# robertvoy/ComfyUI-Distributed

Hardware: AMD Instinct MI355X
Metric: tiles/sec (whole node), sd15 USDU 4x->4096 512px tiles (higher is better)
Workload: dtype bf16; 1 GPU; model=sd15-unet-860M-random-init, global_batch=1, canvas=4096x4096, tile=512+pad32->544, tiles_per_image=64, sampler=euler/20steps/denoise0.5/cfg8.0, parallelism=tile-pull-queue dp1 over RCCL/xGMI

## Files before the change

comfyui_distributed_amd/ops/hip/bindings.cpp:

```cpp
#include <torch/extension.h>

torch::Tensor group_norm_fused(torch::Tensor x, int64_t groups,
                               torch::Tensor weight, torch::Tensor bias,
                               double eps, bool fuse_silu);
torch::Tensor layer_norm_bf16(torch::Tensor x, torch::Tensor gamma,
                              torch::Tensor beta, double eps);
torch::Tensor act_mul_bf16(torch::Tensor a, torch::Tensor b, bool gelu);
torch::Tensor extract_resize(torch::Tensor src, int64_t x1, int64_t y1,
                             int64_t x2, int64_t y2, int64_t ow, int64_t oh);
void blend_tile(torch::Tensor canvas, torch::Tensor tile, int64_t x1,
                int64_t y1, int64_t x2, int64_t y2, int64_t mx1, int64_t my1,
                int64_t mx2, int64_t my2, double sigma);
torch::Tensor attn_fwd(torch::Tensor q, torch::Tensor k, torch::Tensor v,
                       int64_t heads, int64_t kv_heads, int64_t nk_real,
                       double scale);
torch::Tensor attn_fwd_packed(torch::Tensor q, torch::Tensor k,
                              torch::Tensor v, int64_t heads,
                              int64_t kv_heads, double scale);
torch::Tensor attn_fwd_qkv(torch::Tensor qkv, int64_t heads, double scale);
torch::Tensor attn_fwd_q_kv(torch::Tensor q, torch::Tensor kv, int64_t heads,
                            double scale);
torch::Tensor mfma_selftest(torch::Tensor a, torch::Tensor b);
torch::Tensor conv_nhwc(torch::Tensor x, torch::Tensor wt, torch::Tensor bias,
                        int64_t B, int64_t H, int64_t W, int64_t C, int64_t K,
                        int64_t rs, bool fuse_silu);
torch::Tensor group_norm_nhwc(torch::Tensor x, int64_t groups,
                              torch::Tensor weight, torch::Tensor bias,
                              double eps, bool fuse_silu,
                              c10::optional<torch::Tensor> addend);
std::vector<int64_t> group_norm_nhwc_plan(int64_t B, int64_t HW, int64_t C);
torch::Tensor conv_smallc(torch::Tensor x, torch::Tensor wt, torch::Tensor bias,
                          int64_t B, int64_t H, int64_t W, int64_t C,
                          int64_t K, int64_t rs, bool fuse_silu);
torch::Tensor gemm256_bf16(torch::Tensor x, torch::Tensor w,
                           torch::Tensor bias, bool fuse_silu);
torch::Tensor conv256_nhwc(torch::Tensor x, torch::Tensor wt,
                           torch::Tensor bias, torch::Tensor residual,
                           int64_t B, int64_t H,
                           int64_t W, int64_t C, int64_t K, int64_t rs,
                           int64_t stride, bool up2, bool fuse_silu);
torch::Tensor conv256_nhwc_ex(torch::Tensor x, torch::Tensor wt,
                              torch::Tensor bias, torch::Tensor residual,
                              int64_t B, int64_t H,
                              int64_t W, int64_t C, int64_t K, int64_t rs,
                              int64_t stride, bool up2, bool fuse_silu,
                              int64_t bn, int64_t split_k);
std::tuple<int64_t, int64_t> conv256_plan(int64_t M, int64_t K_out,
                                          int64_t Kdim);
void qk_norm_rope(torch::Tensor q, torch::Tensor k, torch::Tensor q_weight,
                  torch::Tensor k_weight, torch::Tensor cos, torch::Tensor sin,
                  torch::Tensor out_q, torch::Tensor out_k, int64_t heads,
                  double eps, int64_t token_offset);
torch::Tensor norm_modulate(torch::Tensor x, torch::Tensor weight,
                            torch::Tensor scale, torch::Tensor shift,
                            double eps);
std::tuple<torch::Tensor, torch::Tensor> norm_modulate_fp8(
    torch::Tensor x, torch::Tensor weight, torch::Tensor scale,
    torch::Tensor shift, double eps);
torch::Tensor gated_residual(torch::Tensor x, torch::Tensor gate,
                             torch::Tensor y);
std::tuple<torch::Tensor, torch::Tensor> quant_rows_fp8(torch::Tensor x);
torch::Tensor gemm_fp8(torch::Tensor qa, torch::Tensor sa, torch::Tensor qw,
                       torch::Tensor sw, torch::Tensor bias, int64_t act);

PYBIND11_MODULE(TORCH_EXTENSION_NAME, m) {
  m.def("group_norm_fused", &group_norm_fused,
        "fused GroupNorm(+SiLU), NCHW bf16");
  m.def("layer_norm", &layer_norm_bf16, "LayerNorm over last dim, bf16");
  m.def("act_mul", &act_mul_bf16, "a * act(b) elementwise, bf16");
  m.def("extract_resize", &extract_resize,
        "crop region of [B,H,W,C] f32 -> Lanczos-3 resample");
  m.def("blend_tile", &blend_tile,
        "fused resample + blurred-rect mask + composite (in-place canvas)");
  m.def("attn_fwd", &attn_fwd, "flash attention forward, bf16 MFMA");
  m.def("attn_fwd_packed", &attn_fwd_packed,
        "flash attention on packed [B,N,H*D] QKV (no host reshapes)");
  m.def("attn_fwd_qkv", &attn_fwd_qkv,
        "self-attention on fused [B,N,3*H*D] projection output");
  m.def("attn_fwd_q_kv", &attn_fwd_q_kv,
        "cross-attention on q [B,Nq,H*D] + fused kv [B,Nk,2*H*D]");
  m.def("mfma_selftest", &mfma_selftest,
        "single-wave 16x16x32 bf16 MFMA with the kernel fragment layouts");
  m.def("conv_nhwc", &conv_nhwc,
        "implicit-GEMM 3x3/1x1 NHWC bf16 conv on MFMA (+fused SiLU)");
  m.def("group_norm_nhwc", &group_norm_nhwc,
        "fused GroupNorm(+SiLU), NHWC bf16; addend [B, C] bf16 is added per "
        "sample (rounded to bf16) before the statistics",
        py::arg("x"), py::arg("groups"), py::arg("weight"), py::arg("bias"),
        py::arg("eps"), py::arg("fuse_silu"), py::arg("addend") = py::none());
  m.def("group_norm_nhwc_plan", &group_norm_nhwc_plan,
        "(B, HW, C) -> (threads, pixels per step, slots per lane, blocks per "
        "image, pixels per block) of the two-pass NHWC GroupNorm; launches "
        "nothing");
  m.def("conv_smallc", &conv_smallc,
        "small-C NHWC conv (stem convs, C <= 8)");
  m.def("gemm256_bf16", &gemm256_bf16,
        "256x256x64 glds-staged MFMA GEMM, torch-Linear layout (+SiLU)");
  m.def("conv256_nhwc", &conv256_nhwc,
        "256-tile implicit-GEMM 3x3/1x1 NHWC conv on the same template; "
        "N-tile width and K split chosen per call");
  m.def("conv256_nhwc_ex", &conv256_nhwc_ex,
        "conv256_nhwc with the variant pinned: bn in {128, 256, 320} and "
        "split_k (clamped to the K-tile count); 0 = chooser");
  m.def("conv256_plan", &conv256_plan,
        "(M, K_out, Kdim) -> (bn, split_k) the conv launcher picks; "
        "launches nothing");
  m.def("qk_norm_rope", &qk_norm_rope,
        "per-head RMSNorm + RoPE of strided q/k views into [B,Ntot,H*D] "
        "buffers at a token offset");
  m.def("norm_modulate", &norm_modulate,
        "row RMSNorm (fp32 weight) or affine-free LayerNorm (empty weight) "
        "+ optional adaLN (1+scale)/shift");
  m.def("norm_modulate_fp8", &norm_modulate_fp8,
        "quant_rows_fp8(norm_modulate(...)) in one launch -> (float8_e4m3fn "
        "[B,N,C], fp32 row scale [B,N]); C % 128 == 0, C <= 8192");
  m.def("gated_residual", &gated_residual, "x + gate[b] * y, bf16");
  m.def("quant_rows_fp8", &quant_rows_fp8,
        "bf16 [M,K] -> (float8_e4m3fn [M,K], fp32 row scale [M] = amax/448)");
  m.def("gemm_fp8", &gemm_fp8,
        "act((qa . qw^T) * sa[m] * sw[n] + bias[n]) -> bf16 on the block-"
        "scaled 16x16x128 MFMA; act 0 none, 1 SiLU, 2 GELU-tanh");
}
```

comfyui_distributed_amd/ops/hip/gemm.hip:

```cpp

#include <torch/extension.h>
#include <ATen/hip/HIPContext.h>
#include "gemm_tile.h"

#define GBM TILE_BM
#define GBN 256
#define GBK 64

struct ConvGeo {
  int H, W, C;
  int Ho, Wo;
  int stride;
  int up2;
  int RS;
  int tile2d;
  int xcd_swz;
};

__device__ __forceinline__ unsigned xcd_remap(unsigned id, unsigned nwg) {
  const unsigned q = nwg / 8u, r = nwg % 8u;
  const unsigned xcd = id % 8u, pos = id / 8u;
  return (xcd < r ? xcd * (q + 1u) : r * (q + 1u) + (xcd - r) * q) + pos;
}

template <bool IS_CONV>
struct AChunk {
  typename std::conditional<IS_CONV, unsigned, long long>::type off;
  int yx;
};
#define A_ROW_DEAD 0x7fff0001

template <bool IS_CONV, bool FUSE_SILU, int BN, bool SPLITK>
__global__ __launch_bounds__(512, 1) void gemm256_kernel(
    const uint16_t* __restrict__ A,
    const uint16_t* __restrict__ Bw,
    const float* __restrict__ bias,
    const uint16_t* __restrict__ zero_page,
    const uint16_t* __restrict__ residual,
    uint16_t* __restrict__ Y,
    float* __restrict__ ws,
    long long M, int N, int Kdim, ConvGeo geo) {
  static_assert(BN == 128 || BN == 256 || BN == 320, "unsupported N-tile");
  constexpr int NF = BN / 64;
  constexpr int NB = BN / 64;
  constexpr unsigned B_TILE = BN * 128u;
  const TileThread t = tile_thread();
  const int wave = t.wave, wm = t.wm, wn = t.wn, fr = t.fr, kgrp = t.kgrp,
            r0 = t.r0;

  __shared__ __align__(16) uint16_t lds[32768 + BN * 128];
  uint8_t* const lds8 = reinterpret_cast<uint8_t*>(lds);

  unsigned bx = blockIdx.x;
  if (IS_CONV && geo.xcd_swz) bx = xcd_remap(bx, gridDim.x);
  long long m_blk = 0;
  int t_b = 0, t_py0 = 0, t_px0 = 0;
  if (IS_CONV && geo.tile2d) {
    const int tx_n = geo.Wo >> 4;
    const int per_img = tx_n * (geo.Ho >> 4);
    t_b = (int)(bx / per_img);
    const int rem = (int)(bx % per_img);
    t_py0 = (rem / tx_n) << 4;
    t_px0 = (rem % tx_n) << 4;
  } else {
    m_blk = (long long)bx * GBM;
  }
  const int n_blk = blockIdx.y * BN;

  const int c_loc = (int)(t.c_byte >> 1);
  const int bn0 = n_blk + r0;
  const long long b_off = (long long)bn0 * Kdim + c_loc;
  AChunk<IS_CONV> a_desc[2][2];
#pragma unroll
  for (int i = 0; i < 2; ++i) {
#pragma unroll
    for (int pc = 0; pc < 2; ++pc) {
      const int m_local = t.a_row(0, pc, i);
      AChunk<IS_CONV> d;
      if (IS_CONV) {
        long long img;
        int py, px;
        bool ok = true;
        if (geo.tile2d) {
          py = t_py0 + (m_local >> 4);
          px = t_px0 + (m_local & 15);
          img = (long long)t_b * geo.H * geo.W * geo.C;
        } else {
          const long long m = m_blk + m_local;
          ok = m < M;
          const long long HWo = (long long)geo.Ho * geo.Wo;
          const long long mm = ok ? m : 0;
          const int pb = (int)(mm / HWo);
          const int rem = (int)(mm - (long long)pb * HWo);
          py = rem / geo.Wo;
          px = rem % geo.Wo;
          img = (long long)pb * geo.H * geo.W * geo.C;
        }
        const long long pix =
            geo.up2 ? 0
                    : ((long long)py * geo.stride * geo.W +
                       (long long)px * geo.stride) * geo.C;
        d.off = img + pix + c_loc;
        d.yx = ok ? ((py * geo.stride + 1) << 16) | (px * geo.stride + 1)
                  : A_ROW_DEAD;
      } else {
        const long long m = m_blk + m_local;
        const bool ok = m < M;
        d.off = (ok ? m * (long long)Kdim : 0) + c_loc;
        d.yx = ok ? 0 : A_ROW_DEAD;
      }
      a_desc[pc][i] = d;
    }
  }

  f32x4_t acc[8][NF];
#pragma unroll
  for (int i = 0; i < 8; ++i)
#pragma unroll
    for (int j = 0; j < NF; ++j) acc[i][j] = f32x4_t{0.f, 0.f, 0.f, 0.f};

  int kt_begin = 0, kt_end = Kdim / GBK;
  if (SPLITK) {
    const int nkt = kt_end, ns = (int)gridDim.z, s = (int)blockIdx.z;
    const int q = nkt / ns, r = nkt % ns;
    kt_begin = s * q + (s < r ? s : r);
    kt_end = kt_begin + q + (s < r ? 1 : 0);
  }

  auto stage_b = [&](int kt, int p, auto J0, auto JN) {
    tile_stage_b<BN == 320, decltype(J0)::value, decltype(JN)::value>(
        Bw, zero_page, b_off, bn0, N, Kdim, kt * GBK,
        lds8 + (unsigned)TILE_BBUF + p * B_TILE, wave);
  };

  auto stage_a = [&](int kt, int p, int pc) {
    const int kbase = kt * GBK;
    uint8_t* const piece =
        lds8 + ((unsigned)TILE_ABUF + p * TILE_IMG + pc * 16384u);
    if constexpr (!IS_CONV) {
      tile_stage_a(A, zero_page,
                   [&](int i, long long& off) {
                     off = a_desc[pc][i].off;
                     return a_desc[pc][i].yx == 0;
                   },
                   kbase, piece, wave);
    } else {
      int tap_dy = 0, tap_dx = 0, cbase = kbase;
      if (geo.RS == 9) {
        const int tap = kbase / geo.C;
        cbase = kbase - tap * geo.C;
        tap_dy = tap / 3 - 1;
        tap_dx = tap % 3 - 1;
      }
      const long long tap_off =
          ((long long)tap_dy * geo.W + tap_dx) * geo.C + cbase;
      const int tap_dq = tap_dy * 65536 + tap_dx;
#pragma unroll
      for (int i = 0; i < 2; ++i) {
        AChunk<IS_CONV> d = a_desc[pc][i];
        if constexpr (BN == 320) {
          asm volatile("" : "+v"(d.off), "+v"(d.yx));
        }
        const int q = d.yx + tap_dq;
        const unsigned ty = (unsigned)(q >> 16) - 1u;
        const unsigned tx = (unsigned)(q & 0xffff) - 1u;
        const uint16_t* src;
        if (geo.up2) {
          const bool ok = ty < 2u * geo.H && tx < 2u * geo.W;
          src = ok ? A + d.off +
                         ((long long)(ty >> 1) * geo.W + (tx >> 1)) * geo.C +
                         cbase
                   : zero_page;
        } else {
          const bool ok = ty < (unsigned)geo.H && tx < (unsigned)geo.W;
          src = ok ? A + d.off + tap_off : zero_page;
        }
        glds16(src, piece + (wave * 64u + i * 512u) * 16u);
      }
    }
  };

  auto compute_cluster = [&](int p, auto MQ, auto NF0, auto NFN, auto KS0,
                             auto KSN) {
    constexpr int mq = decltype(MQ)::value;
    constexpr int nf0 = decltype(NF0)::value;
    constexpr int nfn = decltype(NFN)::value;
    constexpr int ks0 = decltype(KS0)::value;
    constexpr int ksn = decltype(KSN)::value;
    const unsigned a_base = (unsigned)TILE_ABUF + p * TILE_IMG;
    const unsigned b_base = (unsigned)TILE_BBUF + p * B_TILE;
    const int qq = mq * 2 + wm;
    s16x8_t af[4][ksn], bfr[nfn][ksn];
#pragma unroll
    for (int mf = 0; mf < 4; ++mf)
#pragma unroll
      for (int ks = 0; ks < ksn; ++ks) {
        const unsigned lo =
            (qq * 64 + mf * 16 + fr) * 128u + (ks0 + ks) * 64u +
            kgrp * 16u;
        af[mf][ks] = *reinterpret_cast<const s16x8_t*>(
            lds + ((a_base + swz(lo)) >> 1));
      }
#pragma unroll
    for (int nf = 0; nf < nfn; ++nf)
#pragma unroll
      for (int ks = 0; ks < ksn; ++ks) {
        const int brow = wn * (BN / 4) + (nf0 + nf) * 16 + fr;
        const unsigned lo = brow * 128u + (ks0 + ks) * 64u + kgrp * 16u;
        bfr[nf][ks] = *reinterpret_cast<const s16x8_t*>(
            lds + ((b_base + swz(lo)) >> 1));
      }
    __builtin_amdgcn_s_setprio(1);
#pragma unroll
    for (int mf = 0; mf < 4; ++mf)
#pragma unroll
      for (int nf = 0; nf < nfn; ++nf)
#pragma unroll
        for (int ks = 0; ks < ksn; ++ks)
          acc[mq * 4 + mf][nf0 + nf] =
              __builtin_amdgcn_mfma_f32_16x16x32_bf16(
                  bfr[nf][ks], af[mf][ks], acc[mq * 4 + mf][nf0 + nf],
                  0, 0, 0);
    __builtin_amdgcn_s_setprio(0);
  };
  auto cluster = [&](int p, auto MQ, auto NF0, auto NFN) {
    if constexpr (BN == 320) {
      compute_cluster(p, MQ, NF0, NFN, ic<0>{}, ic<1>{});
      compute_cluster(p, MQ, NF0, NFN, ic<1>{}, ic<1>{});
    } else {
      compute_cluster(p, MQ, NF0, NFN, ic<0>{}, ic<2>{});
    }
  };

  stage_b(kt_begin, 0, ic<0>{}, ic<NB>{});
  stage_a(kt_begin, 0, 0);
  stage_a(kt_begin, 0, 1);
  for (int kt = kt_begin; kt < kt_end; ++kt) {
    const int p = (kt - kt_begin) & 1;
    const bool more = kt + 1 < kt_end;
    tile_ktile<BN>(p, kt + 1, more, stage_b, stage_a, cluster);
  }

  const long long m_wave = m_blk + wm * 128;
  const int n_wave = n_blk + wn * (BN / 4);

  const bool vec4 = (N & 3) == 0;

#pragma unroll
  for (int mf = 0; mf < 8; ++mf) {
    long long m;
    if (IS_CONV && geo.tile2d) {
      const int idx = wm * 128 + mf * 16 + fr;
      m = ((long long)t_b * geo.Ho + t_py0 + (idx >> 4)) * geo.Wo + t_px0 +
          (idx & 15);
    } else {
      m = m_wave + mf * 16 + fr;
      if (m >= M) continue;
    }
#pragma unroll
    for (int nf = 0; nf < NF; ++nf) {
      const int n0 = n_wave + nf * 16 + kgrp * 4;
      if (n0 >= N) continue;
      if constexpr (SPLITK) {
        float* dst = ws + ((long long)blockIdx.z * M + m) * N + n0;
        if (vec4) {
          *reinterpret_cast<f32x4_t*>(dst) = acc[mf][nf];
        } else {
#pragma unroll
          for (int c = 0; c < 4; ++c)
            if (n0 + c < N) dst[c] = acc[mf][nf][c];
        }
      } else {
        if (vec4) {
          f32x4_t v = acc[mf][nf];
          if (bias) v += *reinterpret_cast<const f32x4_t*>(bias + n0);
          if (FUSE_SILU) {
#pragma unroll
            for (int c = 0; c < 4; ++c) v[c] = silu_f(v[c]);
          }
          if (residual) {
            const u16x4_t r =
                *reinterpret_cast<const u16x4_t*>(residual + m * N + n0);
#pragma unroll
            for (int c = 0; c < 4; ++c) v[c] += bf16_bits_to_f32(r[c]);
          }
          u16x4_t o;
#pragma unroll
          for (int c = 0; c < 4; ++c) o[c] = f32_to_bf16_bits(v[c]);
          *reinterpret_cast<u16x4_t*>(Y + m * N + n0) = o;
        } else {
#pragma unroll
          for (int c = 0; c < 4; ++c) {
            if (n0 + c >= N) break;
            float v = acc[mf][nf][c] + (bias ? bias[n0 + c] : 0.f);
            if (FUSE_SILU) v = silu_f(v);
            if (residual) v += bf16_bits_to_f32(residual[m * N + n0 + c]);
            Y[m * N + n0 + c] = f32_to_bf16_bits(v);
          }
        }
      }
    }
  }
}

__global__ __launch_bounds__(256) void splitk_reduce_kernel(
    const float* __restrict__ ws,
    const float* __restrict__ bias,
    const uint16_t* __restrict__ residual,
    uint16_t* __restrict__ Y,
    long long M, int N, int S, int fuse_silu) {
  const int ng = (N + 3) >> 2;
  const long long t = (long long)blockIdx.x * blockDim.x + threadIdx.x;
  if (t >= M * ng) return;
  const long long m = t / ng;
  const int n0 = (int)(t - m * ng) * 4;
  const long long slab = M * N;
  const float* src = ws + m * N + n0;
  if ((N & 3) == 0) {
    f32x4_t v = *reinterpret_cast<const f32x4_t*>(src);
    for (int s = 1; s < S; ++s)
      v += *reinterpret_cast<const f32x4_t*>(src + s * slab);
    if (bias) v += *reinterpret_cast<const f32x4_t*>(bias + n0);
    if (fuse_silu) {
#pragma unroll
      for (int c = 0; c < 4; ++c) v[c] = silu_f(v[c]);
    }
    if (residual) {
      const u16x4_t r =
          *reinterpret_cast<const u16x4_t*>(residual + m * N + n0);
#pragma unroll
      for (int c = 0; c < 4; ++c) v[c] += bf16_bits_to_f32(r[c]);
    }
    u16x4_t o;
#pragma unroll
    for (int c = 0; c < 4; ++c) o[c] = f32_to_bf16_bits(v[c]);
    *reinterpret_cast<u16x4_t*>(Y + m * N + n0) = o;
  } else {
    for (int c = 0; c < 4 && n0 + c < N; ++c) {
      float v = src[c];
      for (int s = 1; s < S; ++s) v += src[c + s * slab];
      if (bias) v += bias[n0 + c];
      if (fuse_silu) v = silu_f(v);
      if (residual) v += bf16_bits_to_f32(residual[m * N + n0 + c]);
      Y[m * N + n0 + c] = f32_to_bf16_bits(v);
    }
  }
}


template <bool IS_CONV, int BN>
static void gemm256_launch(dim3 grid, hipStream_t stream, bool fuse_silu,
                           const uint16_t* x, const uint16_t* w,
                           const float* bias, const uint16_t* zero,
                           const uint16_t* res, uint16_t* y, float* ws,
                           long long M, int N, int Kdim, ConvGeo geo) {
  auto go = [&](auto SILU, auto SPLITK) {
    hipLaunchKernelGGL((gemm256_kernel<IS_CONV, decltype(SILU)::value, BN,
                                       decltype(SPLITK)::value>),
                       grid, dim3(512), 0, stream, x, w, bias, zero, res, y,
                       ws, M, N, Kdim, geo);
  };
  if constexpr (IS_CONV) {
    if (grid.z > 1) return go(std::false_type{}, std::true_type{});
  }
  if (fuse_silu) go(std::true_type{}, std::false_type{});
  else go(std::false_type{}, std::false_type{});
}

torch::Tensor gemm256_bf16(torch::Tensor x, torch::Tensor w,
                           torch::Tensor bias, bool fuse_silu) {
  TORCH_CHECK(x.is_cuda() && x.scalar_type() == at::kBFloat16 &&
              x.is_contiguous());
  TORCH_CHECK(w.is_cuda() && w.scalar_type() == at::kBFloat16 &&
              w.is_contiguous());
  const long long M = x.size(0);
  const int K = (int)x.size(1), N = (int)w.size(0);
  TORCH_CHECK(w.size(1) == K && K % GBK == 0, "K must be a multiple of 64");
  auto y = torch::empty({M, (long long)N}, x.options());
  torch::Tensor bf32;
  const float* bptr = bias_f32_ptr(bias, bf32);
  dim3 grid((unsigned)((M + GBM - 1) / GBM), (unsigned)((N + GBN - 1) / GBN));
  auto stream = at::hip::getCurrentHIPStream();
  ConvGeo geo{0, 0, 0, 0, 0, 1, 0, 0, 0, 0};
  gemm256_launch<false, GBN>(
      grid, stream, fuse_silu, (const uint16_t*)x.data_ptr(),
      (const uint16_t*)w.data_ptr(), bptr,
      (const uint16_t*)device_zero_page(x), nullptr, (uint16_t*)y.data_ptr(),
      nullptr, M, N, K, geo);
  HIP_CHECK_LAUNCH();
  return y;
}

static constexpr int kNumCU = 256;
static constexpr double kStepCost128 = 0.70;
static constexpr double kStepCost320 = 1.13;
static constexpr int kMinSliceKtiles = 10;

struct ConvPlan {
  int bn, split_k;
};

static long long conv256_tiles(long long M, int K_out, int bn) {
  return ((M + GBM - 1) / GBM) * (long long)((K_out + bn - 1) / bn);
}

static int conv256_split(long long tiles, int Kdim) {
  if (tiles >= kNumCU) return 1;
  const int nkt = Kdim / GBK;
  return (int)std::max<long long>(
      1, std::min<long long>(kNumCU / tiles, nkt / kMinSliceKtiles));
}

static ConvPlan conv256_choose(long long M, int K_out, int Kdim) {
  const long long t256 = conv256_tiles(M, K_out, 256);
  if (t256 < kNumCU) {
    const int nkt = Kdim / GBK;
    const int s256 = conv256_split(t256, Kdim);
    const int s320 = conv256_split(conv256_tiles(M, K_out, 320), Kdim);
    const double c256 = (nkt + s256 - 1) / s256;
    const double c320 = (nkt + s320 - 1) / s320 * kStepCost320;
    if (s256 > 1 && c320 < 0.95 * c256) return {320, s320};
    return {256, s256};
  }
  auto rounds = [](long long tiles) {
    return (double)((tiles + kNumCU - 1) / kNumCU);
  };
  ConvPlan best{256, 1};
  double cost = rounds(t256);
  const double c320 = rounds(conv256_tiles(M, K_out, 320)) * kStepCost320;
  if (c320 < 0.97 * cost) {
    best = {320, 1};
    cost = c320;
  }
  if (K_out <= 128) {
    const double c128 = rounds(conv256_tiles(M, K_out, 128)) * kStepCost128;
    if (c128 < 0.97 * cost) best = {128, 1};
  }
  return best;
}

std::tuple<int64_t, int64_t> conv256_plan(int64_t M, int64_t K_out,
                                          int64_t Kdim) {
  TORCH_CHECK(M > 0 && K_out > 0 && Kdim > 0 && Kdim % GBK == 0);
  const ConvPlan p = conv256_choose(M, (int)K_out, (int)Kdim);
  return {p.bn, p.split_k};
}

torch::Tensor conv256_nhwc_ex(torch::Tensor x, torch::Tensor wt,
                              torch::Tensor bias, torch::Tensor residual,
                              int64_t B, int64_t H,
                              int64_t W, int64_t C, int64_t K, int64_t rs,
                              int64_t stride, bool up2, bool fuse_silu,
                              int64_t bn, int64_t split_k) {
  TORCH_CHECK(x.is_cuda() && x.scalar_type() == at::kBFloat16 &&
              x.is_contiguous());
  TORCH_CHECK(wt.is_cuda() && wt.is_contiguous());
  TORCH_CHECK(rs == 9 || rs == 1);
  TORCH_CHECK(stride == 1 || (stride == 2 && rs == 9));
  TORCH_CHECK(!up2 || (stride == 1 && rs == 9));
  TORCH_CHECK(C % GBK == 0, "C must be a multiple of 64");
  TORCH_CHECK(bn == 0 || bn == 128 || bn == 256 || bn == 320,
              "bn must be 0, 128, 256 or 320");
  TORCH_CHECK(split_k >= 0, "split_k must be >= 0");
  const int64_t Ho = up2 ? 2 * H : (stride == 1 ? H : (H + 2 - 3) / 2 + 1);
  const int64_t Wo = up2 ? 2 * W : (stride == 1 ? W : (W + 2 - 3) / 2 + 1);
  TORCH_CHECK(H < 16384 && W < 16384, "pixel coords are packed in 16 bits");
  TORCH_CHECK(x.numel() < (1LL << 32), "activation offsets are 32-bit");
  const long long M = B * Ho * Wo;
  const int Kdim = (int)(rs * C);
  TORCH_CHECK(wt.numel() == K * (int64_t)Kdim, "weight must be [K, rs*C]");
  ConvPlan plan = conv256_choose(M, (int)K, Kdim);
  if (bn != 0 && bn != plan.bn)
    plan = {(int)bn,
            conv256_split(conv256_tiles(M, (int)K, (int)bn), Kdim)};
  if (split_k != 0)
    plan.split_k = (int)std::min<int64_t>(split_k, Kdim / GBK);
  auto y = torch::empty({B, Ho, Wo, K}, x.options());
  torch::Tensor bf32;
  const float* bptr = bias_f32_ptr(bias, bf32);
  static const int xcd_swz = [] {
    const char* e = getenv("DISTGPU_CONV_XCDSWZ");
    return (!e || e[0] == '1') ? 1 : 0;
  }();
  const int tile2d = (Ho % 16 == 0 && Wo % 16 == 0) ? 1 : 0;
  const unsigned gx = tile2d
      ? (unsigned)(B * (Ho / 16) * (Wo / 16))
      : (unsigned)((M + GBM - 1) / GBM);
  dim3 grid(gx, (unsigned)((K + plan.bn - 1) / plan.bn),
            (unsigned)plan.split_k);
  auto stream = at::hip::getCurrentHIPStream();
  ConvGeo geo{(int)H, (int)W, (int)C, (int)Ho, (int)Wo, (int)stride,
              up2 ? 1 : 0, (int)rs, tile2d, xcd_swz};
  const uint16_t* resptr = nullptr;
  if (residual.defined() && residual.numel() > 0) {
    TORCH_CHECK(residual.is_cuda() && residual.is_contiguous() &&
                residual.scalar_type() == at::kBFloat16 &&
                residual.numel() == M * K,
                "residual must be a contiguous bf16 [B,Ho,Wo,K] tensor");
    resptr = (const uint16_t*)residual.data_ptr();
  }
  torch::Tensor ws;
  float* wsptr = nullptr;
  if (plan.split_k > 1) {
    ws = torch::empty({(long long)plan.split_k * M * K},
                      x.options().dtype(at::kFloat));
    wsptr = ws.data_ptr<float>();
  }
  const uint16_t* xp = (const uint16_t*)x.data_ptr();
  const uint16_t* wp = (const uint16_t*)wt.data_ptr();
  uint16_t* yp = (uint16_t*)y.data_ptr();
  const uint16_t* zp = (const uint16_t*)device_zero_page(x);
  auto launch = [&](auto BN) {
    gemm256_launch<true, decltype(BN)::value>(grid, stream, fuse_silu, xp, wp,
                                              bptr, zp, resptr, yp, wsptr, M,
                                              (int)K, Kdim, geo);
  };
  if (plan.bn == 128) launch(ic<128>{});
  else if (plan.bn == 320) launch(ic<320>{});
  else launch(ic<256>{});
  HIP_CHECK_LAUNCH();
  if (plan.split_k > 1) {
    const long long nthreads = M * ((K + 3) / 4);
    hipLaunchKernelGGL(splitk_reduce_kernel,
                       dim3((unsigned)((nthreads + 255) / 256)), dim3(256), 0,
                       stream, (const float*)wsptr, bptr, resptr, yp, M,
                       (int)K, plan.split_k, fuse_silu ? 1 : 0);
    HIP_CHECK_LAUNCH();
  }
  return y;
}

torch::Tensor conv256_nhwc(torch::Tensor x, torch::Tensor wt,
                           torch::Tensor bias, torch::Tensor residual,
                           int64_t B, int64_t H,
                           int64_t W, int64_t C, int64_t K, int64_t rs,
                           int64_t stride, bool up2, bool fuse_silu) {
  return conv256_nhwc_ex(x, wt, bias, residual, B, H, W, C, K, rs, stride,
                         up2, fuse_silu, 0, 0);
}
```

comfyui_distributed_amd/ops/hip/gemm_tile.h:

```cpp
#pragma once

#include <type_traits>
#include "common.h"

typedef __attribute__((ext_vector_type(8))) short s16x8_t;
typedef __attribute__((ext_vector_type(4))) int i32x4_t;
typedef __attribute__((ext_vector_type(8))) int i32x8_t;
typedef __attribute__((ext_vector_type(4))) float f32x4_t;
typedef __attribute__((ext_vector_type(4))) uint16_t u16x4_t;

#define TILE_BM 256
#define TILE_ABUF 0
#define TILE_BBUF 65536
#define TILE_IMG 32768

template <int V>
using ic = std::integral_constant<int, V>;

__device__ __forceinline__ unsigned swz(unsigned byte_off) {
  return byte_off ^ (((byte_off >> 9) & 1u) << 5);
}

__device__ __forceinline__ void glds16(const void* gsrc, void* lds_dst) {
  __builtin_amdgcn_global_load_lds(
      (const __attribute__((address_space(1))) uint32_t*)gsrc,
      (__attribute__((address_space(3))) uint32_t*)lds_dst, 16, 0, 0);
}

struct TileThread {
  int lane, wave;
  int wm;
  int wn;
  int fr, kgrp;
  int r0;
  int c_byte;
  template <typename I>
  __device__ __forceinline__ I a_row(I base, int pc, int i) const {
    return base + i * 128 + pc * 64 + r0;
  }
};

__device__ __forceinline__ TileThread tile_thread() {
  TileThread t;
  const int tid = threadIdx.x;
  t.lane = tid & 63;
  t.wave = tid >> 6;
  t.wm = t.wave >> 2;
  t.wn = t.wave & 3;
  t.fr = t.lane & 15;
  t.kgrp = t.lane >> 4;
  const unsigned y0 = swz((unsigned)tid * 16u);
  t.c_byte = (int)(y0 & 127u);
  t.r0 = (int)(y0 >> 7);
  return t;
}


template <bool FENCE, int J0, int JN, typename P>
__device__ __forceinline__ void tile_stage_b(
    const P& Bw, const P& zero_page, const long long& b_off, const int& bn0,
    const int& N, const int& Kdim, int kbase, uint8_t* img, const int& wave) {
  long long b_off_k = b_off;
  if constexpr (FENCE) asm volatile("" : "+v"(b_off_k));
#pragma unroll
  for (int j = J0; j < J0 + JN; ++j) {
    const P src = (bn0 + 64 * j < N)
                      ? Bw + b_off_k + (long long)(64 * j) * Kdim + kbase
                      : zero_page;
    glds16(src, img + (wave * 64u + j * 512u) * 16u);
  }
}

template <typename P, typename Row>
__device__ __forceinline__ void tile_stage_a(const P& A, const P& zero_page,
                                             const Row& row, int kbase,
                                             uint8_t* piece, const int& wave) {
#pragma unroll
  for (int i = 0; i < 2; ++i) {
    long long off;
    const bool live = row(i, off);
    glds16(live ? A + off + kbase : zero_page,
           piece + (wave * 64u + i * 512u) * 16u);
  }
}

template <int BN, typename More, typename StageB, typename StageA,
          typename Cluster>
__device__ __forceinline__ void tile_ktile(int p, int ktn, More more,
                                           const StageB& stage_b,
                                           const StageA& stage_a,
                                           const Cluster& cluster) {
  constexpr int NF = BN / 64;
  constexpr int NB = BN / 64;
  constexpr int NFA = (NF + 1) / 2;
  asm volatile("s_waitcnt vmcnt(0)" ::: "memory");
  __builtin_amdgcn_s_barrier();
  if constexpr (BN == 128) {
    if (more) {
      stage_b(ktn, 1 - p, ic<0>{}, ic<NB>{});
      stage_a(ktn, 1 - p, 0);
    }
    cluster(p, ic<0>{}, ic<0>{}, ic<NF>{});
    if (more) stage_a(ktn, 1 - p, 1);
    cluster(p, ic<1>{}, ic<0>{}, ic<NF>{});
  } else {
    if (more) stage_b(ktn, 1 - p, ic<0>{}, ic<2>{});
    cluster(p, ic<0>{}, ic<0>{}, ic<NFA>{});
    if (more) stage_b(ktn, 1 - p, ic<2>{}, ic<NB - 2>{});
    cluster(p, ic<0>{}, ic<NFA>{}, ic<NF - NFA>{});
    if (more) stage_a(ktn, 1 - p, 0);
    cluster(p, ic<1>{}, ic<0>{}, ic<NFA>{});
    if (more) stage_a(ktn, 1 - p, 1);
    cluster(p, ic<1>{}, ic<NFA>{}, ic<NF - NFA>{});
  }
}
```

Before: 12.75 tiles/s.

## Add stream-K tail scheduling to the 256-tile implicit-GEMM conv

Adds a stream-K mode to the conv GEMM kernel. The first dp_tiles output tiles are computed whole, and the remaining tail tiles are split into per-CU ranges of K-tile steps. Partial accumulators go to an fp32 workspace, and a separate reduce kernel combines them and applies bias, SiLU and the residual. A cost model picks this schedule when it predicts a better wave-quantization fill than the round-counting plan. This targets the partial last wave on a large CU count. The price is an extra launch, workspace traffic, and more complex per-block control flow.

```diff
diff --git a/comfyui_distributed_amd/ops/hip/bindings.cpp b/comfyui_distributed_amd/ops/hip/bindings.cpp
--- a/comfyui_distributed_amd/ops/hip/bindings.cpp
+++ b/comfyui_distributed_amd/ops/hip/bindings.cpp
@@ -47,6 +47,18 @@
                               int64_t bn, int64_t split_k);
 std::tuple<int64_t, int64_t> conv256_plan(int64_t M, int64_t K_out,
                                           int64_t Kdim);
+torch::Tensor conv256_nhwc_sk(torch::Tensor x, torch::Tensor wt,
+                              torch::Tensor bias, torch::Tensor residual,
+                              int64_t B, int64_t H,
+                              int64_t W, int64_t C, int64_t K, int64_t rs,
+                              int64_t stride, bool up2, bool fuse_silu,
+                              int64_t bn, int64_t dp_tiles, int64_t sk_wgs);
+std::tuple<int64_t, int64_t, int64_t, int64_t> conv256_sched(int64_t M,
+                                                             int64_t K_out,
+                                                             int64_t Kdim);
+std::vector<std::tuple<int64_t, int64_t, int64_t, int64_t, int64_t>>
+conv256_sk_segments(int64_t tiles, int64_t kt, int64_t dp_tiles,
+                    int64_t sk_wgs);
 void qk_norm_rope(torch::Tensor q, torch::Tensor k, torch::Tensor q_weight,
                   torch::Tensor k_weight, torch::Tensor cos, torch::Tensor sin,
                   torch::Tensor out_q, torch::Tensor out_k, int64_t heads,
@@ -103,8 +115,17 @@
         "conv256_nhwc with the variant pinned: bn in {128, 256, 320} and "
         "split_k (clamped to the K-tile count); 0 = chooser");
   m.def("conv256_plan", &conv256_plan,
-        "(M, K_out, Kdim) -> (bn, split_k) the conv launcher picks; "
-        "launches nothing");
+        "(M, K_out, Kdim) -> (bn, split_k) of the round-counting plan (the "
+        "one used with the stream-K tail off); launches nothing");
+  m.def("conv256_sched", &conv256_sched,
+        "(M, K_out, Kdim) -> (bn, split_k, dp_tiles, sk_wgs) conv256_nhwc "
+        "runs; sk_wgs = 0: no stream-K tail; launches nothing");
+  m.def("conv256_nhwc_sk", &conv256_nhwc_sk,
+        "conv256_nhwc with the schedule pinned: bn, the first dp_tiles tiles "
+        "whole, the rest cut into sk_wgs ranges of K-tile steps");
+  m.def("conv256_sk_segments", &conv256_sk_segments,
+        "(tiles, kt, dp_tiles, sk_wgs) -> [(range, tile, kt0, kt1, slot)] "
+        "of the stream-K tail, slot -1 = whole tile; launches nothing");
   m.def("qk_norm_rope", &qk_norm_rope,
         "per-head RMSNorm + RoPE of strided q/k views into [B,Ntot,H*D] "
         "buffers at a token offset");
diff --git a/comfyui_distributed_amd/ops/hip/gemm.hip b/comfyui_distributed_amd/ops/hip/gemm.hip
--- a/comfyui_distributed_amd/ops/hip/gemm.hip
+++ b/comfyui_distributed_amd/ops/hip/gemm.hip
@@ -23,6 +23,45 @@
   return (xcd < r ? xcd * (q + 1u) : r * (q + 1u) + (xcd - r) * q) + pos;
 }
 
+struct SkSched {
+  int gx;
+  int kt;
+  int dp_tiles;
+  int sk_wgs;
+  int units;
+  int silu;
+};
+
+struct SkSeg {
+  int tile, kt0, kt1;
+  int slot;
+};
+
+__host__ __device__ inline void sk_range(const SkSched& s, int j, int& b,
+                                         int& e) {
+  const int q = s.units / s.sk_wgs, r = s.units % s.sk_wgs;
+  b = j * q + (j < r ? j : r);
+  e = b + q + (j < r ? 1 : 0);
+}
+
+__host__ __device__ inline int sk_range_of(const SkSched& s, int u) {
+  const int q = s.units / s.sk_wgs, r = s.units % s.sk_wgs;
+  const int head = r * (q + 1);
+  return u < head ? u / (q + 1) : r + (u - head) / q;
+}
+
+__host__ __device__ inline SkSeg sk_segment(const SkSched& s, int j, int u,
+                                            int u_end) {
+  SkSeg g;
+  const int t_rel = u / s.kt;
+  g.tile = s.dp_tiles + t_rel;
+  g.kt0 = u - t_rel * s.kt;
+  const int left = u_end - u;
+  g.kt1 = g.kt0 + left < s.kt ? g.kt0 + left : s.kt;
+  g.slot = (g.kt0 == 0 && g.kt1 == s.kt) ? -1 : j + t_rel;
+  return g;
+}
+
 template <bool IS_CONV>
 struct AChunk {
   typename std::conditional<IS_CONV, unsigned, long long>::type off;
@@ -30,34 +69,41 @@
 };
 #define A_ROW_DEAD 0x7fff0001
 
-template <bool IS_CONV, bool FUSE_SILU, int BN, bool SPLITK>
-__global__ __launch_bounds__(512, 1) void gemm256_kernel(
-    const uint16_t* __restrict__ A,
-    const uint16_t* __restrict__ Bw,
+#define MODE_PLAIN 0
+#define MODE_SPLITK 1
+#define MODE_STREAMK 2
+
+template <bool IS_CONV, bool FUSE_SILU, int BN, int MODE>
+__device__ __forceinline__ void gemm256_tile(
+    const uint16_t* __restrict__ A, const uint16_t* __restrict__ Bw,
     const float* __restrict__ bias,
     const uint16_t* __restrict__ zero_page,
-    const uint16_t* __restrict__ residual,
-    uint16_t* __restrict__ Y,
-    float* __restrict__ ws,
-    long long M, int N, int Kdim, ConvGeo geo) {
+    const uint16_t* __restrict__ residual, uint16_t* __restrict__ Y,
+    float* __restrict__ dst_raw, long long M, int N, int Kdim,
+    const ConvGeo& geo, unsigned bx, unsigned gx, unsigned by, int kt_begin,
+    int kt_end, bool silu_rt) {
   static_assert(BN == 128 || BN == 256 || BN == 320, "unsupported N-tile");
   constexpr int NF = BN / 64;
   constexpr int NB = BN / 64;
   constexpr unsigned B_TILE = BN * 128u;
-  const TileThread t = tile_thread();
+  int tid = threadIdx.x;
+  if constexpr (MODE == MODE_STREAMK) asm volatile("" : "+v"(tid));
+  const TileThread t = tile_thread(tid);
   const int wave = t.wave, wm = t.wm, wn = t.wn, fr = t.fr, kgrp = t.kgrp,
             r0 = t.r0;
 
   __shared__ __align__(16) uint16_t lds[32768 + BN * 128];
   uint8_t* const lds8 = reinterpret_cast<uint8_t*>(lds);
 
-  unsigned bx = blockIdx.x;
-  if (IS_CONV && geo.xcd_swz) bx = xcd_remap(bx, gridDim.x);
+  if (IS_CONV && geo.xcd_swz) bx = xcd_remap(bx, gx);
+  int out_h = geo.Ho, out_w = geo.Wo;
+  if constexpr (MODE == MODE_STREAMK)
+    asm volatile("" : "+s"(out_h), "+s"(out_w));
   long long m_blk = 0;
   int t_b = 0, t_py0 = 0, t_px0 = 0;
   if (IS_CONV && geo.tile2d) {
-    const int tx_n = geo.Wo >> 4;
-    const int per_img = tx_n * (geo.Ho >> 4);
+    const int tx_n = out_w >> 4;
+    const int per_img = tx_n * (out_h >> 4);
     t_b = (int)(bx / per_img);
     const int rem = (int)(bx % per_img);
     t_py0 = (rem / tx_n) << 4;
@@ -65,7 +111,7 @@
   } else {
     m_blk = (long long)bx * GBM;
   }
-  const int n_blk = blockIdx.y * BN;
+  const int n_blk = by * BN;
 
   const int c_loc = (int)(t.c_byte >> 1);
   const int bn0 = n_blk + r0;
@@ -88,12 +134,12 @@
         } else {
           const long long m = m_blk + m_local;
           ok = m < M;
-          const long long HWo = (long long)geo.Ho * geo.Wo;
+          const long long HWo = (long long)out_h * out_w;
           const long long mm = ok ? m : 0;
           const int pb = (int)(mm / HWo);
           const int rem = (int)(mm - (long long)pb * HWo);
-          py = rem / geo.Wo;
-          px = rem % geo.Wo;
+          py = rem / out_w;
+          px = rem % out_w;
           img = (long long)pb * geo.H * geo.W * geo.C;
         }
         const long long pix =
@@ -118,14 +164,6 @@
   for (int i = 0; i < 8; ++i)
 #pragma unroll
     for (int j = 0; j < NF; ++j) acc[i][j] = f32x4_t{0.f, 0.f, 0.f, 0.f};
-
-  int kt_begin = 0, kt_end = Kdim / GBK;
-  if (SPLITK) {
-    const int nkt = kt_end, ns = (int)gridDim.z, s = (int)blockIdx.z;
-    const int q = nkt / ns, r = nkt % ns;
-    kt_begin = s * q + (s < r ? s : r);
-    kt_end = kt_begin + q + (s < r ? 1 : 0);
-  }
 
   auto stage_b = [&](int kt, int p, auto J0, auto JN) {
     tile_stage_b<BN == 320, decltype(J0)::value, decltype(JN)::value>(
@@ -241,28 +279,41 @@
     tile_ktile<BN>(p, kt + 1, more, stage_b, stage_a, cluster);
   }
 
-  const long long m_wave = m_blk + wm * 128;
-  const int n_wave = n_blk + wn * (BN / 4);
+  const int e_row = wm * 128 + fr, e_col = wn * (BN / 4) + kgrp * 4;
 
   const bool vec4 = (N & 3) == 0;
+
+  if constexpr (MODE == MODE_STREAMK) {
+    if (dst_raw) {
+#pragma unroll
+      for (int mf = 0; mf < 8; ++mf)
+#pragma unroll
+        for (int nf = 0; nf < NF; ++nf)
+          *reinterpret_cast<f32x4_t*>(
+              dst_raw + (e_row + mf * 16) * BN + e_col + nf * 16) =
+              acc[mf][nf];
+      return;
+    }
+  }
+  const bool silu = FUSE_SILU || (MODE == MODE_STREAMK && silu_rt);
 
 #pragma unroll
   for (int mf = 0; mf < 8; ++mf) {
     long long m;
     if (IS_CONV && geo.tile2d) {
-      const int idx = wm * 128 + mf * 16 + fr;
-      m = ((long long)t_b * geo.Ho + t_py0 + (idx >> 4)) * geo.Wo + t_px0 +
+      const int idx = e_row + mf * 16;
+      m = ((long long)t_b * out_h + t_py0 + (idx >> 4)) * out_w + t_px0 +
           (idx & 15);
     } else {
-      m = m_wave + mf * 16 + fr;
+      m = m_blk + e_row + mf * 16;
       if (m >= M) continue;
     }
 #pragma unroll
     for (int nf = 0; nf < NF; ++nf) {
-      const int n0 = n_wave + nf * 16 + kgrp * 4;
+      const int n0 = n_blk + e_col + nf * 16;
       if (n0 >= N) continue;
-      if constexpr (SPLITK) {
-        float* dst = ws + ((long long)blockIdx.z * M + m) * N + n0;
+      if constexpr (MODE == MODE_SPLITK) {
+        float* dst = dst_raw + m * N + n0;
         if (vec4) {
           *reinterpret_cast<f32x4_t*>(dst) = acc[mf][nf];
         } else {
@@ -274,7 +325,7 @@
         if (vec4) {
           f32x4_t v = acc[mf][nf];
           if (bias) v += *reinterpret_cast<const f32x4_t*>(bias + n0);
-          if (FUSE_SILU) {
+          if (silu) {
 #pragma unroll
             for (int c = 0; c < 4; ++c) v[c] = silu_f(v[c]);
           }
@@ -293,12 +344,121 @@
           for (int c = 0; c < 4; ++c) {
             if (n0 + c >= N) break;
             float v = acc[mf][nf][c] + (bias ? bias[n0 + c] : 0.f);
-            if (FUSE_SILU) v = silu_f(v);
+            if (silu) v = silu_f(v);
             if (residual) v += bf16_bits_to_f32(residual[m * N + n0 + c]);
             Y[m * N + n0 + c] = f32_to_bf16_bits(v);
           }
         }
       }
+    }
+  }
+}
+
+template <bool IS_CONV, bool FUSE_SILU, int BN, int MODE>
+__global__ __launch_bounds__(512, 1) void gemm256_kernel(
+    const uint16_t* __restrict__ A,
+    const uint16_t* __restrict__ Bw,
+    const float* __restrict__ bias,
+    const uint16_t* __restrict__ zero_page,
+    const uint16_t* __restrict__ residual,
+    uint16_t* __restrict__ Y,
+    float* __restrict__ ws,
+    long long M, int N, int Kdim, ConvGeo geo, SkSched sk) {
+  auto tile = [&](unsigned bx, unsigned gx, unsigned by, int kt_begin,
+                  int kt_end, float* dst_raw) {
+    gemm256_tile<IS_CONV, FUSE_SILU, BN, MODE>(
+        A, Bw, bias, zero_page, residual, Y, dst_raw, M, N, Kdim, geo, bx, gx,
+        by, kt_begin, kt_end, sk.silu != 0);
+  };
+  if constexpr (MODE == MODE_PLAIN) {
+    tile(blockIdx.x, gridDim.x, blockIdx.y, 0, Kdim / GBK, nullptr);
+  } else if constexpr (MODE == MODE_SPLITK) {
+    const int nkt = Kdim / GBK, ns = (int)gridDim.z, s = (int)blockIdx.z;
+    const int q = nkt / ns, r = nkt % ns;
+    const int kt_begin = s * q + (s < r ? s : r);
+    tile(blockIdx.x, gridDim.x, blockIdx.y, kt_begin,
+         kt_begin + q + (s < r ? 1 : 0), ws + (long long)s * M * N);
+  } else {
+    const int w = (int)blockIdx.x;
+    const bool dp = w < sk.dp_tiles;
+    int j = w - sk.dp_tiles;
+    if (!dp && IS_CONV && geo.xcd_swz)
+      j = (int)xcd_remap((unsigned)j, (unsigned)sk.sk_wgs);
+    int u = 0, u_end = sk.kt;
+    if (!dp) sk_range(sk, j, u, u_end);
+    while (u < u_end) {
+      const SkSeg g =
+          dp ? SkSeg{w, 0, sk.kt, -1} : sk_segment(sk, j, u, u_end);
+      tile((unsigned)(g.tile % sk.gx), (unsigned)sk.gx,
+           (unsigned)(g.tile / sk.gx), g.kt0, g.kt1,
+           g.slot < 0 ? nullptr : ws + (long long)g.slot * (GBM * BN));
+      u += g.kt1 - g.kt0;
+      if (u < u_end) {
+        asm volatile("s_waitcnt lgkmcnt(0)" ::: "memory");
+        __builtin_amdgcn_s_barrier();
+      }
+    }
+  }
+}
+
+template <int BN>
+__global__ __launch_bounds__(256) void streamk_reduce_kernel(
+    const float* __restrict__ ws, const float* __restrict__ bias,
+    const uint16_t* __restrict__ residual, uint16_t* __restrict__ Y,
+    long long M, int N, ConvGeo geo, SkSched sk) {
+  constexpr int NG = BN / 4;
+  const long long t = (long long)blockIdx.x * blockDim.x + threadIdx.x;
+  const int cg = (int)(t % NG);
+  const int idx = (int)((t / NG) % GBM);
+  const int t_rel = (int)(t / ((long long)NG * GBM));
+  if (t_rel * sk.kt >= sk.units) return;
+  const int j0 = sk_range_of(sk, t_rel * sk.kt);
+  const int j1 = sk_range_of(sk, (t_rel + 1) * sk.kt - 1);
+  if (j0 == j1) return;
+  const int tile = sk.dp_tiles + t_rel;
+  unsigned bx = (unsigned)(tile % sk.gx);
+  if (geo.xcd_swz) bx = xcd_remap(bx, (unsigned)sk.gx);
+  long long m;
+  if (geo.tile2d) {
+    const int tx_n = geo.Wo >> 4;
+    const int per_img = tx_n * (geo.Ho >> 4);
+    const int rem = (int)(bx % per_img);
+    m = ((long long)(bx / per_img) * geo.Ho + ((rem / tx_n) << 4) +
+         (idx >> 4)) * geo.Wo + ((rem % tx_n) << 4) + (idx & 15);
+  } else {
+    m = (long long)bx * GBM + idx;
+  }
+  const int n0 = (tile / sk.gx) * BN + cg * 4;
+  if (m >= M || n0 >= N) return;
+  const float* src =
+      ws + (long long)(j0 + t_rel) * (GBM * BN) + idx * BN + cg * 4;
+  f32x4_t v = *reinterpret_cast<const f32x4_t*>(src);
+  for (int j = j0 + 1; j <= j1; ++j)
+    v += *reinterpret_cast<const f32x4_t*>(src + (long long)(j - j0) *
+                                                     (GBM * BN));
+  if ((N & 3) == 0) {
+    if (bias) v += *reinterpret_cast<const f32x4_t*>(bias + n0);
+    if (sk.silu) {
+#pragma unroll
+      for (int c = 0; c < 4; ++c) v[c] = silu_f(v[c]);
+    }
+    if (residual) {
+      const u16x4_t r =
+          *reinterpret_cast<const u16x4_t*>(residual + m * N + n0);
+#pragma unroll
+      for (int c = 0; c < 4; ++c) v[c] += bf16_bits_to_f32(r[c]);
+    }
+    u16x4_t o;
+#pragma unroll
+    for (int c = 0; c < 4; ++c) o[c] = f32_to_bf16_bits(v[c]);
+    *reinterpret_cast<u16x4_t*>(Y + m * N + n0) = o;
+  } else {
+    for (int c = 0; c < 4 && n0 + c < N; ++c) {
+      float x = v[c];
+      if (bias) x += bias[n0 + c];
+      if (sk.silu) x = silu_f(x);
+      if (residual) x += bf16_bits_to_f32(residual[m * N + n0 + c]);
+      Y[m * N + n0 + c] = f32_to_bf16_bits(x);
     }
   }
 }
@@ -353,18 +513,21 @@
                            const uint16_t* x, const uint16_t* w,
                            const float* bias, const uint16_t* zero,
                            const uint16_t* res, uint16_t* y, float* ws,
-                           long long M, int N, int Kdim, ConvGeo geo) {
-  auto go = [&](auto SILU, auto SPLITK) {
+                           long long M, int N, int Kdim, ConvGeo geo,
+                           const SkSched* sk = nullptr) {
+  const SkSched sched = sk ? *sk : SkSched{0, 0, 0, 0, 0, 0};
+  auto go = [&](auto SILU, auto MODE) {
     hipLaunchKernelGGL((gemm256_kernel<IS_CONV, decltype(SILU)::value, BN,
-                                       decltype(SPLITK)::value>),
+                                       decltype(MODE)::value>),
                        grid, dim3(512), 0, stream, x, w, bias, zero, res, y,
-                       ws, M, N, Kdim, geo);
+                       ws, M, N, Kdim, geo, sched);
   };
   if constexpr (IS_CONV) {
-    if (grid.z > 1) return go(std::false_type{}, std::true_type{});
-  }
-  if (fuse_silu) go(std::true_type{}, std::false_type{});
-  else go(std::false_type{}, std::false_type{});
+    if (sk) return go(std::false_type{}, ic<MODE_STREAMK>{});
+    if (grid.z > 1) return go(std::false_type{}, ic<MODE_SPLITK>{});
+  }
+  if (fuse_silu) go(std::true_type{}, ic<MODE_PLAIN>{});
+  else go(std::false_type{}, ic<MODE_PLAIN>{});
 }
 
 torch::Tensor gemm256_bf16(torch::Tensor x, torch::Tensor w,
@@ -446,12 +609,96 @@
   return {p.bn, p.split_k};
 }
 
-torch::Tensor conv256_nhwc_ex(torch::Tensor x, torch::Tensor wt,
-                              torch::Tensor bias, torch::Tensor residual,
-                              int64_t B, int64_t H,
-                              int64_t W, int64_t C, int64_t K, int64_t rs,
-                              int64_t stride, bool up2, bool fuse_silu,
-                              int64_t bn, int64_t split_k) {
+static constexpr double kSkSegSteps = 3.0;
+static constexpr double kSkReduceStepsPerMB = 0.17;
+static constexpr double kSkTailStep = 1.15;
+static constexpr double kSkMargin = 0.96;
+static constexpr double kSkMaxFill = 0.85;
+
+struct ConvSched {
+  int bn, split_k;
+  long long dp_tiles;
+  int sk_wgs;
+};
+
+static bool conv256_streamk_enabled() {
+  static const bool on = [] {
+    const char* e = getenv("DISTGPU_CONV_STREAMK");
+    return !e || e[0] == '1';
+  }();
+  return on;
+}
+
+static double conv256_step_cost(int bn) {
+  return bn == 320 ? kStepCost320 : bn == 128 ? kStepCost128 : 1.0;
+}
+
+static ConvSched conv256_sched_choose(long long M, int K_out, int Kdim) {
+  const ConvPlan base = conv256_choose(M, K_out, Kdim);
+  const int nkt = Kdim / GBK;
+  const long long t_base = conv256_tiles(M, K_out, base.bn);
+  ConvSched best{base.bn, base.split_k, t_base, 0};
+  if (!conv256_streamk_enabled() || base.split_k > 1) return best;
+  const double base_cost = (double)((t_base + kNumCU - 1) / kNumCU) * nkt *
+                           conv256_step_cost(base.bn);
+  double cost = kSkMargin * base_cost;
+  const int widths[2] = {base.bn, 320};
+  for (int i = 0; i < (base.bn == 320 || K_out <= 128 ? 1 : 2); ++i) {
+    const int bn = widths[i];
+    const long long tiles = conv256_tiles(M, K_out, bn);
+    const long long R = tiles % kNumCU;
+    if (R == 0 || R > kSkMaxFill * kNumCU) continue;
+    if (tiles < kNumCU && conv256_split(tiles, Kdim) > 1) continue;
+    if (R * nkt / kNumCU < kMinSliceKtiles) continue;
+    const long long L = (R * nkt + kNumCU - 1) / kNumCU;
+    const double step = conv256_step_cost(bn);
+    const double slot_mb = (double)(kNumCU + R - 1) * GBM * bn * 4 / 1e6;
+    const double c = (double)(tiles / kNumCU) * nkt * step +
+                     kSkTailStep * L * step + kSkSegSteps +
+                     kSkReduceStepsPerMB * slot_mb;
+    if (c < cost) {
+      cost = c;
+      best = {bn, 1, tiles - R, kNumCU};
+    }
+  }
+  return best;
+}
+
+std::tuple<int64_t, int64_t, int64_t, int64_t> conv256_sched(int64_t M,
+                                                             int64_t K_out,
+                                                             int64_t Kdim) {
+  TORCH_CHECK(M > 0 && K_out > 0 && Kdim > 0 && Kdim % GBK == 0);
+  const ConvSched s = conv256_sched_choose(M, (int)K_out, (int)Kdim);
+  return {s.bn, s.split_k, s.dp_tiles, s.sk_wgs};
+}
+
+std::vector<std::tuple<int64_t, int64_t, int64_t, int64_t, int64_t>>
+conv256_sk_segments(int64_t tiles, int64_t kt, int64_t dp_tiles,
+                    int64_t sk_wgs) {
+  TORCH_CHECK(tiles > 0 && kt > 0 && dp_tiles >= 0 && dp_tiles <= tiles &&
+              sk_wgs >= 1 && (tiles - dp_tiles) * kt < (1LL << 31));
+  const SkSched s{1, (int)kt, (int)dp_tiles, (int)sk_wgs,
+                  (int)((tiles - dp_tiles) * kt), 0};
+  std::vector<std::tuple<int64_t, int64_t, int64_t, int64_t, int64_t>> out;
+  for (int j = 0; j < s.sk_wgs; ++j) {
+    int u, u_end;
+    sk_range(s, j, u, u_end);
+    while (u < u_end) {
+      const SkSeg g = sk_segment(s, j, u, u_end);
+      TORCH_CHECK(sk_range_of(s, u) == j && sk_range_of(s, u_end - 1) == j);
+      out.emplace_back(j, g.tile, g.kt0, g.kt1, g.slot);
+      u += g.kt1 - g.kt0;
+    }
+  }
+  return out;
+}
+
+template <typename Pick>
+static torch::Tensor conv256_run(torch::Tensor x, torch::Tensor wt,
+                                 torch::Tensor bias, torch::Tensor residual,
+                                 int64_t B, int64_t H, int64_t W, int64_t C,
+                                 int64_t K, int64_t rs, int64_t stride,
+                                 bool up2, bool fuse_silu, const Pick& pick) {
   TORCH_CHECK(x.is_cuda() && x.scalar_type() == at::kBFloat16 &&
               x.is_contiguous());
   TORCH_CHECK(wt.is_cuda() && wt.is_contiguous());
@@ -459,9 +706,6 @@
   TORCH_CHECK(stride == 1 || (stride == 2 && rs == 9));
   TORCH_CHECK(!up2 || (stride == 1 && rs == 9));
   TORCH_CHECK(C % GBK == 0, "C must be a multiple of 64");
-  TORCH_CHECK(bn == 0 || bn == 128 || bn == 256 || bn == 320,
-              "bn must be 0, 128, 256 or 320");
-  TORCH_CHECK(split_k >= 0, "split_k must be >= 0");
   const int64_t Ho = up2 ? 2 * H : (stride == 1 ? H : (H + 2 - 3) / 2 + 1);
   const int64_t Wo = up2 ? 2 * W : (stride == 1 ? W : (W + 2 - 3) / 2 + 1);
   TORCH_CHECK(H < 16384 && W < 16384, "pixel coords are packed in 16 bits");
@@ -469,12 +713,7 @@
   const long long M = B * Ho * Wo;
   const int Kdim = (int)(rs * C);
   TORCH_CHECK(wt.numel() == K * (int64_t)Kdim, "weight must be [K, rs*C]");
-  ConvPlan plan = conv256_choose(M, (int)K, Kdim);
-  if (bn != 0 && bn != plan.bn)
-    plan = {(int)bn,
-            conv256_split(conv256_tiles(M, (int)K, (int)bn), Kdim)};
-  if (split_k != 0)
-    plan.split_k = (int)std::min<int64_t>(split_k, Kdim / GBK);
+  const ConvSched plan = pick(M, Kdim);
   auto y = torch::empty({B, Ho, Wo, K}, x.options());
   torch::Tensor bf32;
   const float* bptr = bias_f32_ptr(bias, bf32);
@@ -506,19 +745,49 @@
                       x.options().dtype(at::kFloat));
     wsptr = ws.data_ptr<float>();
   }
+  SkSched sk{(int)gx, Kdim / GBK, 0, 0, 0, fuse_silu ? 1 : 0};
+  const bool tail = plan.sk_wgs > 0;
+  if (tail) {
+    const long long tiles = (long long)gx * grid.y;
+    const long long R = tiles - plan.dp_tiles;
+    TORCH_CHECK(plan.split_k == 1 && plan.dp_tiles >= 0 && R >= 0,
+                "dp_tiles must be in [0, tiles]");
+    TORCH_CHECK(tiles * sk.kt < (1LL << 31) &&
+                plan.dp_tiles + plan.sk_wgs < (1LL << 31),
+                "schedule units are 32-bit");
+    sk.dp_tiles = (int)plan.dp_tiles;
+    sk.sk_wgs = plan.sk_wgs;
+    sk.units = (int)(R * sk.kt);
+    grid = dim3((unsigned)(plan.dp_tiles + (R > 0 ? plan.sk_wgs : 0)));
+    if (R > 0) {
+      ws = torch::empty({(plan.sk_wgs + R - 1) * (long long)GBM * plan.bn},
+                        x.options().dtype(at::kFloat));
+      wsptr = ws.data_ptr<float>();
+    }
+  }
   const uint16_t* xp = (const uint16_t*)x.data_ptr();
   const uint16_t* wp = (const uint16_t*)wt.data_ptr();
   uint16_t* yp = (uint16_t*)y.data_ptr();
   const uint16_t* zp = (const uint16_t*)device_zero_page(x);
   auto launch = [&](auto BN) {
-    gemm256_launch<true, decltype(BN)::value>(grid, stream, fuse_silu, xp, wp,
-                                              bptr, zp, resptr, yp, wsptr, M,
-                                              (int)K, Kdim, geo);
+    constexpr int bn = decltype(BN)::value;
+    gemm256_launch<true, bn>(grid, stream, fuse_silu, xp, wp, bptr, zp,
+                             resptr, yp, wsptr, M, (int)K, Kdim, geo,
+                             tail ? &sk : nullptr);
+    HIP_CHECK_LAUNCH();
+    if (tail && sk.units > 0) {
+      const long long nthreads =
+          (long long)(sk.units / sk.kt) * GBM * (bn / 4);
+      hipLaunchKernelGGL(streamk_reduce_kernel<bn>,
+                         dim3((unsigned)((nthreads + 255) / 256)), dim3(256),
+                         0, stream, (const float*)wsptr, bptr, resptr, yp, M,
+                         (int)K, geo, sk);
+      HIP_CHECK_LAUNCH();
+    }
   };
   if (plan.bn == 128) launch(ic<128>{});
   else if (plan.bn == 320) launch(ic<320>{});
   else launch(ic<256>{});
-  HIP_CHECK_LAUNCH();
   if (plan.split_k > 1) {
     const long long nthreads = M * ((K + 3) / 4);
     hipLaunchKernelGGL(splitk_reduce_kernel,
@@ -530,6 +799,45 @@
   return y;
 }
 
+torch::Tensor conv256_nhwc_ex(torch::Tensor x, torch::Tensor wt,
+                              torch::Tensor bias, torch::Tensor residual,
+                              int64_t B, int64_t H,
+                              int64_t W, int64_t C, int64_t K, int64_t rs,
+                              int64_t stride, bool up2, bool fuse_silu,
+                              int64_t bn, int64_t split_k) {
+  TORCH_CHECK(bn == 0 || bn == 128 || bn == 256 || bn == 320,
+              "bn must be 0, 128, 256 or 320");
+  TORCH_CHECK(split_k >= 0, "split_k must be >= 0");
+  return conv256_run(
+      x, wt, bias, residual, B, H, W, C, K, rs, stride, up2, fuse_silu,
+      [&](long long M, int Kdim) -> ConvSched {
+        if (bn == 0 && split_k == 0)
+          return conv256_sched_choose(M, (int)K, Kdim);
+        ConvPlan plan = conv256_choose(M, (int)K, Kdim);
+        if (bn != 0 && bn != plan.bn)
+          plan = {(int)bn,
+                  conv256_split(conv256_tiles(M, (int)K, (int)bn), Kdim)};
+        if (split_k != 0)
+          plan.split_k = (int)std::min<int64_t>(split_k, Kdim / GBK);
+        return {plan.bn, plan.split_k, conv256_tiles(M, (int)K, plan.bn), 0};
+      });
+}
+
+torch::Tensor conv256_nhwc_sk(torch::Tensor x, torch::Tensor wt,
+                              torch::Tensor bias, torch::Tensor residual,
+                              int64_t B, int64_t H,
+                              int64_t W, int64_t C, int64_t K, int64_t rs,
+                              int64_t stride, bool up2, bool fuse_silu,
+                              int64_t bn, int64_t dp_tiles, int64_t sk_wgs) {
+  TORCH_CHECK(bn == 128 || bn == 256 || bn == 320,
+              "bn must be 128, 256 or 320");
+  TORCH_CHECK(sk_wgs >= 1 && sk_wgs < (1LL << 30), "sk_wgs must be >= 1");
+  return conv256_run(x, wt, bias, residual, B, H, W, C, K, rs, stride, up2,
+                     fuse_silu, [&](long long, int) -> ConvSched {
+                       return {(int)bn, 1, dp_tiles, (int)sk_wgs};
+                     });
+}
+
 torch::Tensor conv256_nhwc(torch::Tensor x, torch::Tensor wt,
                            torch::Tensor bias, torch::Tensor residual,
                            int64_t B, int64_t H,
diff --git a/comfyui_distributed_amd/ops/hip/gemm_tile.h b/comfyui_distributed_amd/ops/hip/gemm_tile.h
--- a/comfyui_distributed_amd/ops/hip/gemm_tile.h
+++ b/comfyui_distributed_amd/ops/hip/gemm_tile.h
@@ -40,9 +40,8 @@
   }
 };
 
-__device__ __forceinline__ TileThread tile_thread() {
+__device__ __forceinline__ TileThread tile_thread(int tid = threadIdx.x) {
   TileThread t;
-  const int tid = threadIdx.x;
   t.lane = tid & 63;
   t.wave = tid >> 6;
   t.wm = t.wave >> 2;
```

Result: faster. 13.35 tiles/s, median of 6 (+4.8%).
